# KorAP/Datok

Measured on AMD Instinct MI355X. Metric: input MB/s tokenized, tokenizer_de.matok, higher is better.
Workload: dtype u32 table cells, u8 symbol codes; 1 GPU; tokenizer_de.matok, 4096 equal-length 4096 B synthetic German docs per batch (BASELINE.json configs[1]); table_layout=matrix: state-major fused u32 cells, docs_per_gpu=4096, doc_bytes=4096, parallelism=documents sharded over 1 GPU(s), no data-path collective, batches_in_flight=3, inputs=one per batch in flight (generator seeds 2, 3, 4 on rank 0)

## Files before the change

datok_amd/csrc/dtk_batch.cpp:

```cpp
#include <algorithm>
#include <cstdio>
#include <cstring>
#include <memory>

#include "dtk_host.h"

static int alloc_outputs(dtk_batch *b, uint64_t tok, uint64_t sent, uint64_t text) {
  auto grow = [](auto &a, uint64_t n) { return a.fit(n, std::max<uint64_t>(n, 4)); };
  int rc;
  if (tok > b->tok_cap) {
    b->tok_cap = 0;
    if ((rc = grow(b->d_rstart, tok)) || (rc = grow(b->d_rend, tok)) || (rc = grow(b->d_bstart, tok)) ||
        (rc = grow(b->d_bend, tok)) || (rc = grow(b->d_sbefore, tok)))
      return rc;
    b->tok_cap = tok;
  }
  if (sent > b->sent_cap) {
    b->sent_cap = 0;
    if ((rc = grow(b->d_sent, sent))) return rc;
    b->sent_cap = sent;
  }
  if (text > b->text_cap) {
    b->text_cap = 0;
    if ((rc = grow(b->d_ttok, text)) || (rc = grow(b->d_tsent, text)) || (rc = grow(b->d_ts_end, text))) return rc;
// ... 245 lines not shown
  put(b->d_seg_tab, seg_doc.data(), (size_t)ns * 4);
  put(b->d_seg_tab + b->seg_cap, seg_lane0.data(), (size_t)ns * 4);
  put(b->d_seg_tab + 2 * (size_t)b->seg_cap, seg_nl.data(), (size_t)ns * 4);
  put(b->d_seg_tab + 3 * (size_t)b->seg_cap, doc_seg0.data(), ((size_t)nd + 1) * 4);
  put(b->d_lane_doc, lane_doc.data(), lanes * 4);
  put(b->d_chunk_off, chunk_off.data(), ((size_t)nd + 1) * 4);
  { const int rc_ = flush(); if (rc_ != DTK_OK) return rc_; }
  b->n_lanes = (uint32_t)lanes;
  b->plan_valid = true;
  return DTK_OK;
}

DtkSym sym_of(const dtk_batch *b) {
  const dtk_model *m = b->last_model;
  return DtkSym{b->d_sym, (m && m->sig.n_codes) ? m->sig.code_entry : nullptr};
}

DtkWalkArgs walk_args(dtk_batch *b) {
  DtkWalkArgs w{};
  w.sym = sym_of(b); w.doc_off = b->d_off; w.n_docs = b->n_docs;
  w.bits = b->d_bits; w.bit_words = b->bit_words; w.doc_tail = b->d_doc_tail; w.status = b->d_status;
  w.tok_cnt = b->d_tok_cnt; w.sent_cnt = b->d_sent_cnt; w.text_cnt = b->d_text_cnt;
  w.steps = (unsigned long long *)dtk_step_stripe(b->d_totals, 0);
  w.step_factor = 2048;
  return w;
}

static DtkSpecArgs spec_args(dtk_batch *b, bool redo) {
  DtkSpecArgs s{};
  s.n_lanes = b->n_lanes; s.chunk = b->chunk; s.warm = b->cfg_warm;
  s.lane_doc = b->d_lane_doc; s.chunk_off = b->d_chunk_off;
  s.lane_start = b->d_lane_start; s.lane_end = b->d_lane_end; s.lane_plan = b->d_lane_plan;
  s.lane_cnt = b->d_lane_cnt; s.first_bad = b->d_first_bad; s.fail_lane = b->d_fail_lane;
  s.redo_from = redo ? b->d_redo : nullptr;
  s.text = b->d_text;
  s.warm_extend = b->cfg_extend;
  const bool lds = g_dbg.lds_bits != 0;
  s.lds_words = (lds && b->chunk <= DTK_LDS_BIT_CHUNK_MAX) ? DTK_LDS_BIT_WORDS(b->chunk) : 0u;
  return s;
}

static uint32_t *n_bad_now(dtk_batch *b) { return b->d_totals->n_bad + b->dev_rounds; }

static int reread_flags(dtk_batch *b) {
  HIP_TRY(hipMemcpyAsync(&b->h_totals->any_irregular, &b->d_totals->any_irregular, 8, hipMemcpyDeviceToHost, b->stream));
  HIP_TRY(hipStreamSynchronize(b->stream));
  return DTK_OK;
}

static uint32_t cmp_mask_of(const dtk_model *m) {
  return LANE_F_SENT | LANE_F_TEXT | (m->unknown_used ? LANE_F_OK : 0u);
}

static int launch_compact2(dtk_batch *b, int which) {
  DtkCompactArgs a = b->last_args;
  set_outputs(b, a);
  a.tok_cap = b->tok_cap; a.sent_cap = b->sent_cap; a.text_cap = b->text_cap;
  const bool seg = b->chunk != 0 && b->long_docs;
  a.seg_doc = seg ? b->d_seg_tab : nullptr;
  a.seg_lane0 = b->d_seg_tab + b->seg_cap; a.seg_nl = b->d_seg_tab + 2 * (size_t)b->seg_cap;
  a.n_segs = b->n_segs; a.chunk_off = b->d_chunk_off; a.lane_start = b->d_lane_start; a.lane_cnt = b->d_lane_cnt;
  a.seg_sum = b->d_seg_sum; a.seg_in = b->d_seg_in;
  a.doc_seq = b->d_seg_tab + 3 * (size_t)b->seg_cap + b->max_docs + 1;
  a.any_irregular = &b->d_totals->any_irregular;
  a.any_eot = &b->d_totals->any_eot;
  b->last_args = a;
  if (seg && (which & 1) && dtk_launch_seg_prepare(&a, b->d_seg_tab + 3 * (size_t)b->seg_cap, b->stream))
    return hip_fail(hipGetLastError(), "segment carries");
  if (dtk_launch_compact(&a, b->small_max, b->d_big_docs, b->n_big, which, b->stream))
    return hip_fail(hipGetLastError(), "compact pass 2");
  if (which & 2) b->ran_full = true;
  return DTK_OK;
}

static int repair_round(dtk_batch *b, const dtk_model *m, const DtkWalkArgs *w, const DtkSpecArgs *sp, uint32_t *n_bad_out) {
  hipStream_t s = b->stream;
  if (dtk_launch_spec(&m->tab, w, sp, 5, cmp_mask_of(m), b->d_redo, n_bad_out, s) ||
      dtk_launch_redo_clear(w, sp, s))
    return hip_fail(hipGetLastError(), "speculative repair");
  for (int stage = 1; stage <= 4; stage++)
    if (dtk_launch_spec(&m->tab, w, sp, stage, cmp_mask_of(m), b->d_redo, n_bad_out, s))
      return hip_fail(hipGetLastError(), "speculative repair");
  return DTK_OK;
}


extern "C" int dtk_batch_run(const dtk_model *m, dtk_batch *b, uint32_t flags) {
  if (!m || !b) return DTK_E_ARG;
  if (b->n_docs == 0 || !b->d_off) return DTK_E_STATE;
  if (m->device != b->device) return DTK_E_ARG;
  int prc = plan_lanes(b);
  if (prc != DTK_OK) return prc;
  if (b->dl_begun && !b->dl_waited) { HIP_TRY(hipEventSynchronize(b->ev_dl)); b->dl_waited = true; }
  b->dl_begun = false;
  b->blk_pending = b->blk_failed = 0;
  b->evl_pending = false; b->evl_need = 0;
  if (b->up_pending) {
    HIP_TRY(hipStreamWaitEvent(b->stream, b->ev_up, 0));
    b->up_pending = false;
  }
  b->last_model = m;
  b->last_flags = flags;
  b->repair_rounds = 0;
  hipStream_t s = b->stream;
  const bool prof = b->profiling;
#define STAGE(i) do { if (prof) HIP_TRY(hipEventRecord(b->ev[i], s)); } while (0)
  STAGE(0);
  bool fold_acc = false;
  size_t acc_bytes = 0;
  {
    const size_t nd = b->n_docs;
    uint8_t *q = b->d_acc;
    b->d_tok_off = b->d_csr; b->d_sent_off = b->d_csr + (nd + 1); b->d_text_off = b->d_csr + 2 * (nd + 1);
    b->d_totals = (DtkTotalsDev *)q; q += DTK_TOTALS_BYTES;
    b->d_tok_cnt = (uint64_t *)q; q += (nd + 1) * 8;
    b->d_sent_cnt = (uint64_t *)q; q += (nd + 1) * 8;
    b->d_text_cnt = (uint64_t *)q; q += (nd + 1) * 8;
    b->d_status = (uint32_t *)q; q += nd * 4;
    b->d_first_bad = (uint32_t *)q; q += nd * 4;
    b->d_fail_lane = (uint32_t *)q; q += nd * 4;
    b->d_doc_tail = (uint32_t *)q; q += nd * 4;
    const size_t acc_used = ((size_t)(q - b->d_acc) + 15) & ~(size_t)15;
    b->bit_words = (uint32_t)(((b->total + nd) / 32 + 8) & ~(uint64_t)3);
    const bool fold = b->total > 0;
    fold_acc = fold && b->acc_primed && acc_used / 16 < 0xFFFFFFFFull && !g_dbg.clear_kernel;
    if (!fold_acc) {
      if (dtk_launch_clear2(b->d_acc, acc_used, b->d_bits, fold ? 0 : (size_t)EVB_KINDS * b->bit_words * 4, s))
        return hip_fail(hipGetLastError(), "clear");
      b->acc_primed = true;
    }
    acc_bytes = acc_used;
  }
  STAGE(1);
  if (dtk_launch_symbolize(b->d_text, b->d_off, b->n_docs, b->total, &m->sig, b->d_sym,
                           b->d_text == b->d_text_own, b->d_blk_doc, (unsigned long long *)&b->d_totals->invalid_epoch,
                           (uint32_t *)b->d_rsbits.p, b->d_bits, b->bit_words, fold_acc ? b->d_acc.p : nullptr, acc_bytes,
                           ++b->epoch, s))
    return hip_fail(hipGetLastError(), "symbolize");
  STAGE(2);
  DtkWalkArgs w = walk_args(b);
  bool fix_in_scan = false;
  DtkSpecArgs sp_first{};
  if (b->chunk == 0) {
    STAGE(3); STAGE(4);
    if (dtk_launch_walk(&m->tab, &w, s)) return hip_fail(hipGetLastError(), "walk");
    STAGE(5); STAGE(6); STAGE(7);
  } else {
    DtkSpecArgs sp = spec_args(b, false);
    sp_first = sp;
    uint32_t *nb = b->d_totals->n_bad;
    const bool split = g_dbg.split_start != 0 || sp.lds_words == 0;
    b->dev_rounds = g_dbg.dev_rounds >= 0 ? (uint32_t)g_dbg.dev_rounds : (b->expect_repairs ? 2u : 0u);
    if (b->dev_rounds > 3u) b->dev_rounds = 3u;
    fix_in_scan = b->n_docs <= 8192u && b->dev_rounds == 0;
#define SPEC(stage)                                                                               \
  do {                                                                                            \
    if (dtk_launch_spec(&m->tab, &w, &sp, stage, cmp_mask_of(m), b->d_redo, nb, s))               \
      return hip_fail(hipGetLastError(), "speculative walk");                                     \
  } while (0)
    if (split) {
      SPEC(0); STAGE(3); SPEC(1); STAGE(4); SPEC(2); STAGE(5); SPEC(3); STAGE(6);
    } else {
      STAGE(3); STAGE(4); SPEC(6); STAGE(5); SPEC(7); STAGE(6);
    }
    if (!fix_in_scan) SPEC(4);
    STAGE(7);
#undef SPEC
    for (uint32_t r = 0; r < b->dev_rounds; r++) {
      DtkSpecArgs rp = spec_args(b, true);
      rp.go = nb + r;
      int rc = repair_round(b, m, &w, &rp, nb + r + 1);
      if (rc != DTK_OK) return rc;
    }
  }
  DtkCompactArgs c{};
  c.text = b->d_text; c.rs_bits = (const uint32_t *)b->d_rsbits.p; c.doc_off = b->d_off; c.n_docs = b->n_docs;
  c.bits = b->d_bits; c.bit_words = b->bit_words; c.doc_tail = b->d_doc_tail; c.status = b->d_status;
  c.flags = flags & DTK_NEWLINE_AFTER_EOT; c.kind = m->kind;
  c.totals = &b->d_totals->n_tok;
  if (dtk_launch_scan3(b->d_tok_cnt, b->d_sent_cnt, b->d_text_cnt, b->d_tok_off, b->d_sent_off, b->d_text_off,
                       b->n_docs, &b->d_totals->n_tok, b->d_status, b->d_scan_ws, fix_in_scan ? &sp_first : nullptr, b->d_redo,
                       b->d_totals->n_bad, b->chunk ? n_bad_now(b) : nullptr, s))
    return hip_fail(hipGetLastError(), "scan");
  STAGE(8);
  c.skip_if = b->chunk ? n_bad_now(b) : nullptr;
  b->last_args = c;
  b->ran_full = false;
  const bool eager_full = g_dbg.compact_full != 0;
  int rc = launch_compact2(b, (b->expect_eot || eager_full) ? 3 : 1);
  if (rc != DTK_OK) return rc;
  STAGE(9);
#undef STAGE
  b->eager_fields = 0;
  b->results_changed = false;
  if (b->fields & DTK_R_EAGER) {
    rc = launch_to_host(b);
    if (rc != DTK_OK) return rc;
  }
  HIP_TRY(hipMemcpyAsync(b->h_totals, b->d_totals, DTK_TOTALS_BYTES, hipMemcpyDeviceToHost, s));
  if ((rc = b->ev_ran.ensure(hipEventDisableTiming)) != DTK_OK) return rc;
  HIP_TRY(hipEventRecord(b->ev_ran, s));
  b->ev_ran_valid = true;
  b->ran = true;
  b->totals_valid = false;
  b->render_flags = 0xFFFFFFFFu;
  return DTK_OK;
}

extern "C" int dtk_batch_done(dtk_batch *b) {
  if (!b || !b->ran || !b->ev_ran) return 0;
  const hipError_t e = hipEventQuery(b->ev_ran);
  if (e != hipSuccess) (void)hipGetLastError();
  return e == hipSuccess ? 1 : 0;
}

extern "C" int dtk_batch_set_profiling(dtk_batch *b, int enable) {
  if (!b) return DTK_E_ARG;
  if (enable)
    for (Event &e : b->ev)
      if (const int rc = e.ensure(hipEventDefault)) return rc;
  b->profiling = enable != 0;
  return DTK_OK;
}

extern "C" int dtk_batch_stage_ms(dtk_batch *b, float ms[DTK_N_STAGES]) {
  if (!b || !ms) return DTK_E_ARG;
  if (!b->ran || !b->profiling) return DTK_E_STATE;
  HIP_TRY(hipStreamSynchronize(b->stream));
  for (int i = 0; i < DTK_N_STAGES; i++) HIP_TRY(hipEventElapsedTime(&ms[i], b->ev[i], b->ev[i + 1]));
  return DTK_OK;
}

extern "C" int dtk_batch_sync(dtk_batch *b) {
  if (!b) return DTK_E_ARG;
  return wait_own(b);
}

static int run_exact(dtk_batch *b) {
  const dtk_model *m = b->last_model;
  hipStream_t s = b->stream;
  const uint32_t nd = b->n_docs;
  std::vector<uint32_t> st(nd);
  HIP_TRY(hipMemcpy(st.data(), b->d_status, (size_t)nd * 4, hipMemcpyDeviceToHost));
  for (uint32_t d = 0; d < nd; d++)
    if (st[d] & ST_IRREGULAR) b->h_exact_ids.push_back(d);
  const uint32_t n = (uint32_t)b->h_exact_ids.size();
  if (n == 0) return DTK_OK;
  if (n > b->exact_cap) {
    const uint64_t cap = (uint64_t)n + n / 4 + 16;
    int rc;
    b->exact_cap = 0;
    if ((rc = b->d_exact_ids.fit(cap, cap)) || (rc = b->d_exact_cnt.fit(cap, cap)) || (rc = b->d_exact_off.fit(cap + 1, cap + 1)))
      return rc;
    b->exact_cap = (uint32_t)cap;
  }
  HIP_TRY(hipMemcpy(b->d_exact_ids, b->h_exact_ids.data(), (size_t)n * 4, hipMemcpyHostToDevice));
  DtkExactArgs X{};
  X.sym = sym_of(b); X.text = b->d_text; X.doc_off = b->d_off; X.n = n; X.docs = b->d_exact_ids;
  X.n_calls = b->d_exact_cnt; X.call_off = b->d_exact_off; X.status = b->d_status;
  X.flags = b->last_flags & DTK_NEWLINE_AFTER_EOT; X.step_factor = walk_args(b).step_factor;
  set_outputs(b, X);
  X.pass = 0;
  if (dtk_launch_exact(&m->tab, &X, s)) return hip_fail(hipGetLastError(), "exact pass (count)");
  std::vector<uint32_t> cnt(n);
  HIP_TRY(hipMemcpyAsync(cnt.data(), b->d_exact_cnt, (size_t)n * 4, hipMemcpyDeviceToHost, s));
  HIP_TRY(hipStreamSynchronize(s));
  b->h_exact_off.assign((size_t)n + 1, 0);
  for (uint32_t i = 0; i < n; i++) b->h_exact_off[i + 1] = b->h_exact_off[i] + cnt[i];
  const uint64_t total = b->h_exact_off[n];
  if (const int rc = b->d_calls.fit(total, total + total / 4 + 16)) return rc;
  HIP_TRY(hipMemcpy(b->d_exact_off, b->h_exact_off.data(), ((size_t)n + 1) * 8, hipMemcpyHostToDevice));
  X.calls = b->d_calls;
  X.pass = 1;
  if (dtk_launch_exact(&m->tab, &X, s)) return hip_fail(hipGetLastError(), "exact pass");
  b->h_calls.resize((size_t)total);
  if (total) HIP_TRY(hipMemcpyAsync(b->h_calls.data(), b->d_calls, (size_t)total * sizeof(DtkCall), hipMemcpyDeviceToHost, s));
  HIP_TRY(hipMemcpyAsync(st.data(), b->d_status, (size_t)nd * 4, hipMemcpyDeviceToHost, s));
  HIP_TRY(hipStreamSynchronize(s));
  uint64_t flagged = 0;
  for (uint32_t d = 0; d < nd; d++) flagged += st[d] != 0;
  b->h_totals->n_flagged = flagged;
  return DTK_OK;
}

int finish(dtk_batch *b) {
  if (!b->ran) return DTK_E_STATE;
  if (b->totals_valid) return DTK_OK;
  { const int rc_ = wait_own(b); if (rc_ != DTK_OK) return rc_; }
  if (b->chunk != 0) {
    const uint32_t *hnb = b->h_totals->n_bad;
    for (uint32_t r = 0; r < b->dev_rounds; r++)
      if (hnb[r] != 0) b->repair_rounds++;
    uint32_t left = hnb[b->dev_rounds];
    if (left != 0) {
      b->results_changed = true;
      const dtk_model *m = b->last_model;
      hipStream_t s = b->stream;
      DtkWalkArgs w = walk_args(b);
      uint32_t *n_bad = n_bad_now(b);
      const uint32_t max_rounds = b->max_doc_lanes + 16u;
      while (left != 0) {
        b->repair_rounds++;
        DtkSpecArgs sp = spec_args(b, true);
        HIP_TRY(hipMemsetAsync(n_bad, 0, 4, s));
        int rc = repair_round(b, m, &w, &sp, n_bad);
        if (rc != DTK_OK) return rc;
        HIP_TRY(hipMemcpyAsync(&left, n_bad, 4, hipMemcpyDeviceToHost, s));
// ... 131 lines not shown
```

datok_amd/csrc/dtk_compact.hip:

```cpp
#include "dtk_device.h"


#define CQ_CAP 512u
#define CT_CAP 512u

struct SegRange { uint32_t d, p0, p1; bool first, last; };
__device__ __forceinline__ bool seg_range(const DtkCompactArgs &A, uint32_t s, uint32_t len_of_d, SegRange &r) {
  const uint32_t La = A.seg_lane0[s], Lb = La + A.seg_nl[s];
  const uint32_t L0 = A.chunk_off[r.d], L1 = A.chunk_off[r.d + 1];
  r.first = La == L0;
  r.last = Lb >= L1;
  r.p0 = r.first ? 0u : A.lane_start[La].p;
  if (r.p0 == 0xFFFFFFFFu) return false;
  r.p1 = r.last ? len_of_d : A.lane_start[Lb].p;
  if (r.p1 == 0xFFFFFFFFu) { r.p1 = len_of_d; r.last = true; }
  return true;
}

__device__ __forceinline__ uint32_t bits32(const uint32_t *__restrict__ b, uint32_t bit) {
  const uint32_t w = bit >> 5, sh = bit & 31u;
  const uint32_t lo = b[w], hi = b[w + 1];
  return (uint32_t)((((uint64_t)hi << 32) | lo) >> sh);
}
__device__ __forceinline__ uint32_t lowmask(uint32_t n) { return n >= 32u ? 0xFFFFFFFFu : (1u << n) - 1u; }
// ... 572 lines not shown
  for (uint32_t q0 = 0; q0 <= len; q0 += 32u) {
    const uint32_t valid = lowmask(len + 1u - q0);
    const uint32_t wE = nE & valid, wS = nS & valid, wP = nP & valid, wT = nT & valid, wU = nU & valid;
    const uint32_t wR = q0 < len ? nR & lowmask(len - q0) : 0u;
    {
      const uint32_t q1 = q0 + 32u <= len ? q0 + 32u : q0;
      nE = bits32(bE, gb + q1); nS = bits32(bS, gb + q1); nP = bits32(bP, gb + q1);
      nT = bits32(bT, gb + q1); nU = bits32(bU, gb + q1);
      nR = bits32(A.rs_bits, (uint32_t)off + (q1 < len ? q1 : 0u));
    }
    uint32_t ev = wE | wP | wT;
    while (ev) {
      const uint32_t b = (uint32_t)__ffs((int)ev) - 1u, m = 1u << b;
      ev &= ev - 1u;
      const uint32_t p = q0 + b, R = Rw + (uint32_t)__popc(wR & lowmask(b));
      if (wT & m) {
        if (wU & m) sentence_end();
        text_end();
        if (is_matrix) { B = p; RB = R; }
      }
      if (wE & m) {
        const uint32_t ms = wS & lowmask(b);
        if (ms) {
          const uint32_t sb = 31u - (uint32_t)__clz((int)ms);
          cs = q0 + sb; Rcs = Rw + (uint32_t)__popc(wR & lowmask(sb));
        }
        if (posC == 0 && nl_rule && p > B && txt[B] == '\n' && !init) posC--;
        init = false;
        posC += (int32_t)(Rcs - RB);
        const int32_t rs = posC;
        if (sentB) {
          sentB = false;
          if (n_sent < sent_n) A.sent[sent_base + n_sent] = rs; else st |= ST_INTERNAL;
          n_sent++;
        }
        posC += (int32_t)(R - Rcs);
        last_rend = posC;
        if (n_tok < tok_n) {
          if (A.tok_bstart) { A.tok_bstart[tok_base + n_tok] = cs; A.tok_bend[tok_base + n_tok] = p; }
          if (A.tok_rstart) { A.tok_rstart[tok_base + n_tok] = rs; A.tok_rend[tok_base + n_tok] = posC; }
          if (A.tok_sbefore) A.tok_sbefore[tok_base + n_tok] = n_sev;
        } else st |= ST_INTERNAL;
        n_tok++;
        B = p; RB = R;
      }
      if (wP & m) sentence_end();
    }
    if (wS) {
      const uint32_t sb = 31u - (uint32_t)__clz((int)wS);
      cs = q0 + sb; Rcs = Rw + (uint32_t)__popc(wR & lowmask(sb));
    }
    Rw += (uint32_t)__popc(wR);
  }
  if (tw & DTK_TAIL_S) sentence_end();
  if (tw & DTK_TAIL_E) text_end();
  if (st || n_tok != tok_n || n_sent != sent_n || n_text != text_n) {
    atomicOr(&A.status[d], ST_IRREGULAR);
    atomicOr(A.any_irregular, 1u);
  }
  if (A.doc_ns) A.doc_ns[d] = n_sev;
}


__device__ __forceinline__ uint32_t wave_sum(uint32_t v) {
#pragma unroll
  for (int o = 32; o > 0; o >>= 1) v += __shfl_xor(v, o);
  return v;
}

__device__ __forceinline__ uint32_t runes_between(const uint32_t *__restrict__ bits, uint64_t g0, uint64_t g1) {
  uint32_t n = 0;
  if (g1 > g0) {
    const uint64_t w0 = g0 >> 5, wl = (g1 - 1) >> 5;
    for (uint64_t w = w0 + lane_id(); w <= wl; w += WAVE) {
      uint32_t x = bits[w];
      if (w == w0) x &= 0xFFFFFFFFu << (g0 & 31u);
      if (w == wl && (g1 & 31u)) x &= (1u << (g1 & 31u)) - 1u;
      n += (uint32_t)__popc(x);
    }
  }
  return wave_sum(n);
}

__global__ __launch_bounds__(WAVE) void k_seg_sum(DtkCompactArgs A) {
  const uint32_t s = blockIdx.x;
  if (s >= A.n_segs) return;
  if (A.skip_if && *A.skip_if != 0u) return;
  const uint32_t d = A.seg_doc[s];
  if (A.chunk_off[d + 1] - A.chunk_off[d] <= DTK_SEG_LANES) return;
  const uint64_t off = A.doc_off[d];
  const uint32_t len = (uint32_t)(A.doc_off[d + 1] - off);
  const uint32_t lane = lane_id();
  DtkSegSum o{0u, 0u, 0u, 0u, 0u, 0xFFFFFFFFu, 0u, 0u};
  SegRange sr{d, 0u, len, true, true};
  if (seg_range(A, s, len, sr)) {
    const uint32_t La = A.seg_lane0[s], nl = A.seg_nl[s];
    DtkLaneCount c{0u, 0u, 0u, 0u, 0u, 0xFFFFFFFFu, 0u, 0u};
    if (lane < nl) c = A.lane_cnt[La + lane];
    uint32_t tot;
    const uint32_t tok_before = wave_excl_scan(c.tok, tot);
    o.tok = tot;
    o.sent = wave_sum(c.sent); o.text = wave_sum(c.text); o.sev = wave_sum(c.sev);
    o.runes = runes_between(A.rs_bits, off + sr.p0, off + sr.p1);
    const unsigned long long mE = __ballot(c.e_pos != 0xFFFFFFFFu);
    if (mE) {
      const int j = highest(mE);
      o.e_pos = __shfl(c.e_pos, j);
      o.e_tok = __shfl(tok_before + c.e_tok, j);
      o.e_runes = runes_between(A.rs_bits, off + sr.p0, off + o.e_pos);
    }
  }
  if (lane == 0) A.seg_sum[s] = o;
}

__global__ __launch_bounds__(WAVE) void k_seg_scan(DtkCompactArgs A, const uint32_t *doc_seg0) {
  const uint32_t d = blockIdx.x;
  if (d >= A.n_docs) return;
  if (A.skip_if && *A.skip_if != 0u) return;
  const uint32_t s0 = doc_seg0[d], s1 = doc_seg0[d + 1];
  if (s1 - s0 <= 1u) return;
  const uint32_t lane = lane_id();
  bool any_e = false;
  uint32_t bt = 0, bs = 0, bx = 0, bv = 0, br = 0;
  uint32_t ce_pos = 0xFFFFFFFFu, ce_tok = 0, ce_runes = 0;
  for (uint32_t g = s0; g < s1; g += WAVE) {
    const uint32_t s = g + lane;
    DtkSegSum v{0u, 0u, 0u, 0u, 0u, 0xFFFFFFFFu, 0u, 0u};
    if (s < s1) v = A.seg_sum[s];
    uint32_t tt, ts, tx, tv, tr;
    const uint32_t et = wave_excl_scan(v.tok, tt), es = wave_excl_scan(v.sent, ts), ex = wave_excl_scan(v.text, tx);
    const uint32_t ev = wave_excl_scan(v.sev, tv), er = wave_excl_scan(v.runes, tr);
    const unsigned long long mE = __ballot(v.e_pos != 0xFFFFFFFFu);
    const unsigned long long below = mE & lanemask_lt();
    const int j = below ? highest(below) : 0;
    const uint32_t jp = __shfl(v.e_pos, j), jt = __shfl(bt + et + v.e_tok, j), jr = __shfl(br + er + v.e_runes, j);
    if (s < s1) {
      DtkSegIn in;
      in.tok = bt + et; in.sent = bs + es; in.text = bx + ex; in.sev = bv + ev; in.runes = br + er;
      in.e_pos = below ? jp : ce_pos; in.e_tok = below ? jt : ce_tok; in.e_runes = below ? jr : ce_runes;
      A.seg_in[s] = in;
    }
    if (mE) {
      const int jl = highest(mE);
      ce_pos = __shfl(v.e_pos, jl); ce_tok = __shfl(bt + et + v.e_tok, jl); ce_runes = __shfl(br + er + v.e_runes, jl);
      any_e = true;
    }
    bt += tt; bs += ts; bx += tx; bv += tv; br += tr;
  }
  if (lane == 0) A.doc_seq[d] = (A.kind != DTK_KIND_MATRIX && any_e) ? 1u : 0u;
}



#define SCAN1_TB 1024u
__global__ __launch_bounds__(SCAN1_TB) void k_scan3(const uint64_t *ca, const uint64_t *cb, const uint64_t *cc,
                                                uint64_t *a, uint64_t *b, uint64_t *c, uint32_t n,
                                                uint64_t *totals, const uint32_t *status, DtkSpecArgs S,
                                                uint32_t *redo_out, uint32_t *n_bad, int fix, const uint32_t *skip_if) {
  if (skip_if && *skip_if != 0u) return;
  __shared__ uint64_t wsum[3][SCAN1_TB / WAVE];
  __shared__ uint32_t wfl[SCAN1_TB / WAVE];
  const uint32_t T = blockDim.x, tid = threadIdx.x, lane = tid & 63u, wid = tid >> 6;
  const uint32_t per = (n + T - 1) / T;
  const uint32_t lo = tid * per < n ? tid * per : n;
  const uint32_t hi = lo + per < n ? lo + per : n;
  uint64_t sa = 0, sb = 0, sc = 0;
  uint32_t fl = 0;
  constexpr uint32_t G = 4u;
  for (uint32_t i0 = lo; i0 < hi; i0 += G) {
    uint64_t va[G], vb[G], vc[G];
    uint32_t vs[G], vf[G];
#pragma unroll
    for (uint32_t j = 0; j < G; j++) {
      const uint32_t i = i0 + j;
      const bool ok = i < hi;
      va[j] = ok ? ca[i] : 0ull; vb[j] = ok ? cb[i] : 0ull; vc[j] = ok ? cc[i] : 0ull;
      vs[j] = ok ? status[i] : 0u;
      vf[j] = (ok && fix) ? S.fail_lane[i] : 0u;
    }
#pragma unroll
    for (uint32_t j = 0; j < G; j++) {
      sa += va[j]; sb += vb[j]; sc += vc[j]; fl += vs[j] != 0u;
      if (fix && i0 + j < hi) {
        const uint32_t bad = ~vf[j];
        if (bad == 0xFFFFFFFFu) redo_out[i0 + j] = 0xFFFFFFFFu; else mark_redo(S, i0 + j, bad, redo_out, n_bad);
      }
    }
  }
  uint64_t xa = sa, xb = sb, xc = sc;
  uint32_t xf = fl;
#pragma unroll
  for (int o = 1; o < WAVE; o <<= 1) {
    const uint64_t ya = __shfl_up(xa, o), yb = __shfl_up(xb, o), yc = __shfl_up(xc, o);
    const uint32_t yf = __shfl_up(xf, o);
    if ((int)lane >= o) { xa += ya; xb += yb; xc += yc; xf += yf; }
  }
  if (lane == WAVE - 1) { wsum[0][wid] = xa; wsum[1][wid] = xb; wsum[2][wid] = xc; wfl[wid] = xf; }
  __syncthreads();
  uint64_t ba = 0, bb = 0, bc = 0;
  uint32_t bf = 0;
  for (uint32_t w = 0; w < wid; w++) { ba += wsum[0][w]; bb += wsum[1][w]; bc += wsum[2][w]; bf += wfl[w]; }
  uint64_t ra = ba + xa - sa, rb = bb + xb - sb, rc = bc + xc - sc;
  for (uint32_t i0 = lo; i0 < hi; i0 += G) {
    uint64_t va[G], vb[G], vc[G];
#pragma unroll
    for (uint32_t j = 0; j < G; j++) {
      const uint32_t i = i0 + j;
      const bool ok = i < hi;
      va[j] = ok ? ca[i] : 0ull; vb[j] = ok ? cb[i] : 0ull; vc[j] = ok ? cc[i] : 0ull;
    }
#pragma unroll
    for (uint32_t j = 0; j < G; j++) {
      const uint32_t i = i0 + j;
      if (i < hi) { a[i] = ra; b[i] = rb; c[i] = rc; }
      ra += va[j]; rb += vb[j]; rc += vc[j];
    }
  }
  if (tid == T - 1) {
    a[n] = ba + xa; b[n] = bb + xb; c[n] = bc + xc;
    totals[0] = ba + xa; totals[1] = bb + xb; totals[2] = bc + xc;
    totals[3] = bf + xf;
  }
}

#ifndef DTK_TOHOST_WAVES
#define DTK_TOHOST_WAVES 128u
#endif
__global__ __launch_bounds__(WAVE) void k_to_host(DtkToHostArgs A) {
  if (A.skip_if && *A.skip_if != 0u) return;
  bool fits = true;
  for (uint32_t i = 0; i < A.n; i++)
    if (A.count_from[i] >= 0 && A.totals[A.count_from[i]] > A.cap[i]) fits = false;
  if (!fits) return;
  const uint32_t lane = threadIdx.x;
  for (uint32_t i = 0; i < A.n; i++) {
    const uint64_t bytes = A.count_from[i] >= 0 ? A.totals[A.count_from[i]] * A.bytes[i] : A.bytes[i];
    const uint4 *__restrict__ s16 = reinterpret_cast<const uint4 *>(A.src[i]);
    uint4 *__restrict__ d16 = reinterpret_cast<uint4 *>(A.dst[i]);
    const uint64_t n16 = bytes >> 4;
    for (uint64_t p = (blockIdx.x + gridDim.x - i % gridDim.x) % gridDim.x; p * WAVE < n16; p += gridDim.x) {
      const uint64_t j = p * WAVE + lane;
      if (j < n16) {
        const uint4 v = s16[j];
        d16[j] = v;
      }
      asm volatile("s_waitcnt vmcnt(0)" ::: "memory");
    }
    if (blockIdx.x == i % gridDim.x && lane < (bytes & 15u))
      reinterpret_cast<uint8_t *>(A.dst[i])[(n16 << 4) + lane] = reinterpret_cast<const uint8_t *>(A.src[i])[(n16 << 4) + lane];
  }
  if (blockIdx.x == 0 && lane == 0) *A.done = A.epoch;
}

extern "C" int dtk_launch_to_host(const DtkToHostArgs *args, void *stream) {
  hipLaunchKernelGGL(k_to_host, dim3(DTK_TOHOST_WAVES), dim3(WAVE), 0, (hipStream_t)stream, *args);
  return (int)hipGetLastError();
}

__global__ __launch_bounds__(256) void k_pack_r16(const int32_t *__restrict__ rs, const int32_t *__restrict__ re,
                                                  uint32_t *__restrict__ out, uint64_t n) {
  const uint64_t i4 = ((uint64_t)blockIdx.x * 256u + threadIdx.x) * 4u;
  if (i4 + 4u <= n) {
    const int4 a = *reinterpret_cast<const int4 *>(rs + i4), b = *reinterpret_cast<const int4 *>(re + i4);
    *reinterpret_cast<uint4 *>(out + i4) =
        make_uint4(((uint32_t)a.x & 0xFFFFu) | ((uint32_t)b.x << 16), ((uint32_t)a.y & 0xFFFFu) | ((uint32_t)b.y << 16),
                   ((uint32_t)a.z & 0xFFFFu) | ((uint32_t)b.z << 16), ((uint32_t)a.w & 0xFFFFu) | ((uint32_t)b.w << 16));
  } else {
    for (uint64_t i = i4; i < n; i++) out[i] = ((uint32_t)rs[i] & 0xFFFFu) | ((uint32_t)re[i] << 16);
  }
}

extern "C" int dtk_launch_pack_r16(const int32_t *rs, const int32_t *re, uint32_t *out, uint64_t n, void *stream) {
  if (n == 0) return 0;
  hipLaunchKernelGGL(k_pack_r16, dim3((unsigned)((n + 1023u) / 1024u)), dim3(256), 0, (hipStream_t)stream, rs, re, out, n);
  return (int)hipGetLastError();
}

__global__ __launch_bounds__(256) void k_pack_blk(DtkPackBlkArgs A) {
  const DtkPackBlkPair P = A.pair[blockIdx.y];
  const uint32_t lane = lane_id();
  const uint64_t blk = (uint64_t)blockIdx.x * 4u + (threadIdx.x >> 6);
  if (blk * WAVE >= A.n) return;
  const uint64_t i = blk * WAVE + lane;
  const bool live = i < A.n;
  int32_t s = 0, e = 0;
  if (live) { s = P.start[i]; e = P.end[i]; }
  const int32_t prev_e = __shfl_up(e, 1);
  const unsigned long long dec = __ballot(live && lane != 0u && s < prev_e);
  const uint32_t brk = dec ? (uint32_t)__ffsll((long long)dec) - 1u : (uint32_t)WAVE;
  const bool seg1 = lane >= brk;
  const int32_t lo = live ? min(s, e) : INT32_MAX, hi = live ? max(s, e) : INT32_MIN;
  const int32_t lo0 = wave_min(seg1 ? INT32_MAX : lo), hi0 = wave_max(seg1 ? INT32_MIN : hi);
  int32_t lo1 = 0, hi1 = 0;
  if (brk < WAVE) { lo1 = wave_min(seg1 ? lo : INT32_MAX); hi1 = wave_max(seg1 ? hi : INT32_MIN); }
  const int32_t base = seg1 ? lo1 : lo0;
  if (live) P.words[i] = ((uint32_t)(s - base) & 0xFFFFu) | ((uint32_t)(e - base) << 16);
  if (lane == 0u) {
    reinterpret_cast<uint4 *>(P.heads)[blk] = make_uint4((uint32_t)lo0, (uint32_t)lo1, brk, 0u);
    if ((int64_t)hi0 - lo0 > (int64_t)A.span || (int64_t)hi1 - lo1 > (int64_t)A.span) atomicOr(P.flag, 1u);
  }
}

extern "C" int dtk_launch_pack_blk(const DtkPackBlkArgs *args, void *stream) {
  if (args->n == 0 || args->n_pairs == 0) return 0;
  const uint64_t blocks = (args->n + WAVE - 1) / WAVE;
  hipLaunchKernelGGL(k_pack_blk, dim3((unsigned)((blocks + 3u) / 4u), args->n_pairs), dim3(256), 0, (hipStream_t)stream, *args);
  return (int)hipGetLastError();
}


__global__ __launch_bounds__(256) void k_clear2(uint4 *__restrict__ a, uint64_t na16, uint4 *__restrict__ b,
                                                uint64_t nb16) {
  const uint64_t stride = (uint64_t)gridDim.x * blockDim.x;
  const uint4 z = make_uint4(0u, 0u, 0u, 0u);
  for (uint64_t i = (uint64_t)blockIdx.x * blockDim.x + threadIdx.x; i < na16 + nb16; i += stride) {
    if (i < na16) a[i] = z; else b[i - na16] = z;
  }
}

extern "C" int dtk_launch_clear2(void *a, uint64_t a_bytes, void *b, uint64_t b_bytes, void *stream) {
  const uint64_t n16 = (a_bytes + b_bytes) / 16;
  if (n16 == 0) return 0;
  uint64_t blocks = (n16 + 256ull * 4 - 1) / (256ull * 4);
  if (blocks > 8192) blocks = 8192;
  hipLaunchKernelGGL(k_clear2, dim3((uint32_t)blocks), dim3(256), 0, (hipStream_t)stream, (uint4 *)a, a_bytes / 16,
                     (uint4 *)b, b_bytes / 16);
  return (int)hipGetLastError();
}

extern "C" int dtk_launch_compact(const DtkCompactArgs *args, uint32_t small_max, const uint32_t *big_docs, uint32_t n_big,
                                  int which, void *stream) {
  if (args->n_docs == 0) return 0;
  hipStream_t s = (hipStream_t)stream;
  if (small_max && (which & 1))
    hipLaunchKernelGGL(k_compact_small, dim3((args->n_docs + 255u) / 256u), dim3(256), 0, s, *args, small_max);
  const uint32_t grid = args->seg_doc ? args->n_segs : (small_max ? n_big : args->n_docs);
  const uint32_t *list = args->seg_doc ? nullptr : (small_max ? big_docs : nullptr);
  if (grid && (which & 1)) hipLaunchKernelGGL(k_compact_plain, dim3(grid), dim3(WAVE), 0, s, *args, small_max, list);
  if (grid && (which & 2)) hipLaunchKernelGGL(k_compact_eot, dim3(grid), dim3(WAVE), 0, s, *args, small_max, list);
  return (int)hipGetLastError();
}

extern "C" int dtk_launch_seg_prepare(const DtkCompactArgs *args, const uint32_t *doc_seg0, void *stream) {
  hipStream_t s = (hipStream_t)stream;
  hipLaunchKernelGGL(k_seg_sum, dim3(args->n_segs), dim3(WAVE), 0, s, *args);
  hipLaunchKernelGGL(k_seg_scan, dim3(args->n_docs), dim3(WAVE), 0, s, *args, doc_seg0);
  return (int)hipGetLastError();
}

#define SCAN_TB 256u
#define SCAN_PER 8u
#define SCAN_TILE (SCAN_TB * SCAN_PER)

__device__ __forceinline__ uint64_t scan_block_excl(uint64_t v, uint64_t *sh, uint64_t &total) {
  const uint32_t tid = threadIdx.x;
  sh[tid] = v;
  __syncthreads();
  for (uint32_t o = 1; o < SCAN_TB; o <<= 1) {
    const uint64_t x = tid >= o ? sh[tid - o] : 0;
    __syncthreads();
    sh[tid] += x;
    __syncthreads();
  }
  total = sh[SCAN_TB - 1];
  const uint64_t ex = sh[tid] - v;
  __syncthreads();
  return ex;
}

__global__ __launch_bounds__(SCAN_TB) void k_scan3_sums(const uint64_t *ca, const uint64_t *cb, const uint64_t *cc,
                                                        const uint32_t *status, uint32_t n, uint64_t *ws, const uint32_t *skip_if) {
  if (skip_if && *skip_if != 0u) return;
  __shared__ uint64_t sh[SCAN_TB];
  const uint32_t i0 = blockIdx.x * SCAN_TILE + threadIdx.x * SCAN_PER;
  uint64_t s[4] = {0, 0, 0, 0};
  for (uint32_t i = i0; i < i0 + SCAN_PER && i < n; i++) { s[0] += ca[i]; s[1] += cb[i]; s[2] += cc[i]; s[3] += status[i] != 0; }
  for (int j = 0; j < 4; j++) {
    uint64_t tot;
    (void)scan_block_excl(s[j], sh, tot);
    if (threadIdx.x == 0) ws[4u * blockIdx.x + j] = tot;
  }
}

__global__ __launch_bounds__(SCAN_TB) void k_scan3_mid(uint64_t *ws, uint32_t nb, uint64_t *a, uint64_t *b, uint64_t *c,
                                                       uint32_t n, uint64_t *totals, const uint32_t *skip_if) {
  if (skip_if && *skip_if != 0u) return;
  __shared__ uint64_t sh[SCAN_TB];
  const uint32_t tid = threadIdx.x;
  const uint32_t per = (nb + SCAN_TB - 1) / SCAN_TB;
  const uint32_t lo = min(tid * per, nb), hi = min(lo + per, nb);
  for (int j = 0; j < 4; j++) {
    uint64_t sm = 0;
    for (uint32_t i = lo; i < hi; i++) sm += ws[4u * i + j];
    uint64_t tot;
    uint64_t run = scan_block_excl(sm, sh, tot);
    for (uint32_t i = lo; i < hi; i++) { const uint64_t v = ws[4u * i + j]; ws[4u * i + j] = run; run += v; }
    if (tid == 0) {
      totals[j] = tot;
      if (j == 0) a[n] = tot;
      if (j == 1) b[n] = tot;
      if (j == 2) c[n] = tot;
    }
  }
}

__global__ __launch_bounds__(SCAN_TB) void k_scan3_apply(const uint64_t *ca, const uint64_t *cb, const uint64_t *cc,
                                                         uint64_t *a, uint64_t *b, uint64_t *c, uint32_t n,
                                                         const uint64_t *ws, const uint32_t *skip_if) {
  if (skip_if && *skip_if != 0u) return;
  __shared__ uint64_t sh[SCAN_TB];
  const uint32_t i0 = blockIdx.x * SCAN_TILE + threadIdx.x * SCAN_PER;
  const uint64_t *src[3] = {ca, cb, cc};
  uint64_t *dst[3] = {a, b, c};
  for (int j = 0; j < 3; j++) {
    uint64_t v[SCAN_PER], sm = 0;
    for (uint32_t q = 0; q < SCAN_PER; q++) { v[q] = i0 + q < n ? src[j][i0 + q] : 0; sm += v[q]; }
    uint64_t tot;
    uint64_t run = ws[4u * blockIdx.x + j] + scan_block_excl(sm, sh, tot);
    for (uint32_t q = 0; q < SCAN_PER; q++) {
      if (i0 + q < n) dst[j][i0 + q] = run;
      run += v[q];
    }
  }
}

extern "C" int dtk_launch_scan3(const uint64_t *ca, const uint64_t *cb, const uint64_t *cc, uint64_t *a,
                                uint64_t *b, uint64_t *c, uint32_t n_docs, uint64_t *totals,
                                const uint32_t *status, uint64_t *ws, const DtkSpecArgs *fix_spec,
                                uint32_t *redo_out, uint32_t *n_bad, const uint32_t *skip_if, void *stream) {
  hipStream_t s = (hipStream_t)stream;
  if (n_docs <= 8192u || !ws) {
    DtkSpecArgs none{};
    hipLaunchKernelGGL(k_scan3, dim3(1), dim3(SCAN1_TB), 0, s, ca, cb, cc, a, b, c, n_docs, totals, status,
                       fix_spec ? *fix_spec : none, redo_out, n_bad, fix_spec ? 1 : 0, skip_if);
  } else {
    if (fix_spec) return -1;
    const uint32_t nb = (n_docs + SCAN_TILE - 1) / SCAN_TILE;
    hipLaunchKernelGGL(k_scan3_sums, dim3(nb), dim3(SCAN_TB), 0, s, ca, cb, cc, status, n_docs, ws, skip_if);
    hipLaunchKernelGGL(k_scan3_mid, dim3(1), dim3(SCAN_TB), 0, s, ws, nb, a, b, c, n_docs, totals, skip_if);
    hipLaunchKernelGGL(k_scan3_apply, dim3(nb), dim3(SCAN_TB), 0, s, ca, cb, cc, a, b, c, n_docs, ws, skip_if);
  }
  return (int)hipGetLastError();
}
```

datok_amd/csrc/dtk_device.h:

```cpp
#pragma once
#include <hip/hip_runtime.h>
#include <stdint.h>

#include <type_traits>

#include "dtk_internal.h"

#define WAVE 64
#ifndef DTK_WARM_TAG
#define DTK_WARM_TAG 64u
#endif


__device__ __forceinline__ uint32_t lane_id() { return threadIdx.x & (WAVE - 1); }
__device__ __forceinline__ unsigned long long lanemask_lt() { return (1ull << lane_id()) - 1ull; }
__device__ __forceinline__ int highest(unsigned long long m) { return 63 - __clzll((long long)m); }
__device__ __forceinline__ uint32_t popc(unsigned long long m) { return (uint32_t)__popcll(m); }

__device__ __forceinline__ uint32_t wave_excl_scan(uint32_t v, uint32_t &total) {
  uint32_t x = v;
  x += (uint32_t)__builtin_amdgcn_update_dpp(0, (int)x, 0x111, 0xF, 0xF, true);
  x += (uint32_t)__builtin_amdgcn_update_dpp(0, (int)x, 0x112, 0xF, 0xF, true);
  x += (uint32_t)__builtin_amdgcn_update_dpp(0, (int)x, 0x114, 0xF, 0xF, true);
  x += (uint32_t)__builtin_amdgcn_update_dpp(0, (int)x, 0x118, 0xF, 0xF, true);
  x += (uint32_t)__builtin_amdgcn_update_dpp(0, (int)x, 0x142, 0xA, 0xF, false);
  x += (uint32_t)__builtin_amdgcn_update_dpp(0, (int)x, 0x143, 0xC, 0xF, false);
  total = (uint32_t)__builtin_amdgcn_readlane((int)x, WAVE - 1);
  return x - v;
}

#define DTK_WAVE_FOLD(x, op)                                                                   \
  do {                                                                                         \
    x = op(x, __builtin_amdgcn_update_dpp(x, x, 0x111, 0xF, 0xF, false));       \
    x = op(x, __builtin_amdgcn_update_dpp(x, x, 0x112, 0xF, 0xF, false));       \
    x = op(x, __builtin_amdgcn_update_dpp(x, x, 0x114, 0xF, 0xF, false));       \
    x = op(x, __builtin_amdgcn_update_dpp(x, x, 0x118, 0xF, 0xF, false));       \
    x = op(x, __builtin_amdgcn_update_dpp(x, x, 0x142, 0xA, 0xF, false));    \
    x = op(x, __builtin_amdgcn_update_dpp(x, x, 0x143, 0xC, 0xF, false));    \
  } while (0)
__device__ __forceinline__ int32_t wave_min(int32_t v) {
  int x = v;
  DTK_WAVE_FOLD(x, min);
  return __builtin_amdgcn_readlane(x, WAVE - 1);
}
__device__ __forceinline__ int32_t wave_max(int32_t v) {
  int x = v;
  DTK_WAVE_FOLD(x, max);
  return __builtin_amdgcn_readlane(x, WAVE - 1);
}

__device__ __forceinline__ uint32_t doc_of(const uint64_t *__restrict__ doc_off, uint32_t lo, uint32_t hi,
                                           uint64_t g) {
  while (hi - lo > 1) {
    const uint32_t mid = lo + ((hi - lo) >> 1);
    if (doc_off[mid] <= g) lo = mid; else hi = mid;
  }
  return lo;
}

__device__ __forceinline__ void mark_redo(const DtkSpecArgs &S, uint32_t d, uint32_t bad, uint32_t *redo_out,
                                          uint32_t *n_bad) {
  const uint32_t L0 = S.chunk_off[d], L1 = S.chunk_off[d + 1];
  DtkLaneState en = S.lane_end[bad];
  en.flags &= (LANE_F_SENT | LANE_F_TEXT | LANE_F_OK);
  if (en.p != 0xFFFFFFFFu && bad + 1 < L1) S.lane_start[bad + 1] = en;
  uint32_t r0 = bad;
  if (bad > L0) {
    r0 = bad - 1u;
    while (r0 > L0 && S.lane_end[r0].p == S.lane_start[r0].p) r0--;
  }
  redo_out[d] = r0;
  atomicAdd(n_bad, 1u);
}
```

datok_amd/csrc/dtk_internal.h:

```cpp
#pragma once
#include <stddef.h>
#include <stdint.h>

#define DTK_FIRSTBIT 0x80000000u
#define DTK_SECONDBIT 0x40000000u
#define DTK_RESTBIT 0x3fffffffu
#define DTK_EOT 4u
#define DTK_WINDOW 1024u
#define DTK_WINDOW_BYTES 4104u

#define DTK_SYM_MASK 0x7FFu
#define DTK_SYM_MAX 2047u
#define DTK_SYM_W_SHIFT 11
#define DTK_SYM_CLS_SHIFT 14
#define DTK_SYM_WIDTH(e) (((uint32_t)(e) >> DTK_SYM_W_SHIFT) & 7u)
#define DTK_SYM_IS_START(e) (DTK_SYM_WIDTH(e) != 0u)
#define DTK_WIN 32u
#define DTK_WIN_ROW 36u
#define DTK_SYM_CONT 0xFFu
#ifndef DTK_WIN8
#define DTK_WIN8 32u
#endif
#ifndef DTK_WIN16
#define DTK_WIN16 16u
// ... 166 lines not shown
  uint32_t flags;
  int kind;
  uint64_t *tok_off, *sent_off, *text_off;
  int32_t *tok_rstart, *tok_rend;
  uint32_t *tok_bstart, *tok_bend;
  int32_t *sent;
  uint32_t *text_tok_end, *text_sent_end;
  uint32_t *tok_sbefore, *text_s_end, *doc_ns;
  const uint64_t *totals;
  uint64_t tok_cap, sent_cap, text_cap;
  const uint32_t *seg_doc, *seg_lane0, *seg_nl;
  uint32_t n_segs;
  const uint32_t *chunk_off;
  const struct DtkLaneState *lane_start;
  const struct DtkLaneCount *lane_cnt;
  struct DtkSegSum *seg_sum;
  struct DtkSegIn *seg_in;
  uint32_t *doc_seq;
  uint32_t *any_irregular;
  uint32_t *any_eot;
  const uint32_t *skip_if;
};

#define DTK_SEG_LANES 64u
struct DtkSegSum {
  uint32_t tok, sent, text, sev;
  uint32_t runes;
  uint32_t e_pos;
  uint32_t e_tok, e_runes;
};
struct DtkSegIn {
  uint32_t tok, sent, text, sev, runes;
  uint32_t e_pos, e_tok, e_runes;
};

struct DtkCall { uint32_t kind; int32_t a; uint32_t b, c; };
struct DtkExactArgs {
  struct DtkSym sym;
  const uint8_t *text;
  const uint64_t *doc_off;
  uint32_t n;
  const uint32_t *docs;
  uint32_t pass;
  uint32_t *n_calls;
  const uint64_t *call_off;
  struct DtkCall *calls;
  uint32_t *status;
  uint32_t flags;
  uint32_t step_factor;
  const uint64_t *tok_off, *sent_off, *text_off;
  int32_t *tok_rstart, *tok_rend;
  uint32_t *tok_bstart, *tok_bend;
  int32_t *sent;
  uint32_t *text_tok_end, *text_sent_end;
  uint32_t *tok_sbefore, *text_s_end, *doc_ns;
};

struct DtkRenderArgs {
  const uint8_t *text;
  const uint64_t *doc_off;
  uint32_t n_docs;
  uint32_t flags;
  const uint64_t *tok_off, *sent_off, *text_off;
  uint64_t n_tok, n_sent, n_text;
  const int32_t *rstart, *rend, *sent;
  const uint32_t *bstart, *bend, *sbefore;
  const uint32_t *ttok, *tsent, *ts_end;
  const uint32_t *doc_ns;
  struct DtkSym sym;
  uint64_t *A, *P, *Q;
  uint64_t *blkA, *blkP, *blkQ;
  uint64_t *ns_off;
  uint64_t *tx_base, *tx_stream, *tx_pos, *tx_sent;
  uint64_t *out_off;
  uint8_t *out;
  uint64_t out_total;
};

#define DTK_TOHOST_MAX 14
struct DtkToHostArgs {
  const void *src[DTK_TOHOST_MAX];
  void *dst[DTK_TOHOST_MAX];
  uint64_t bytes[DTK_TOHOST_MAX];
  int32_t count_from[DTK_TOHOST_MAX];
  uint64_t cap[DTK_TOHOST_MAX];
  uint32_t n;
  const uint64_t *totals;
  const uint32_t *skip_if;
  uint64_t *done;
  uint64_t epoch;
};

struct DtkPackBlkPair {
  const int32_t *start, *end;
  uint32_t *words;
  void *heads;
  uint32_t *flag;
};
struct DtkPackBlkArgs {
  struct DtkPackBlkPair pair[2];
  uint32_t n_pairs;
  uint32_t span;
  uint64_t n;
};

#define DTK_EVL_K_SEOT 1u
#define DTK_EVL_K_TEOT 2u
#define DTK_EVL_K_SEPS 4u
struct DtkEvListArgs {
  const uint32_t *bits;
  uint32_t bit_words;
  uint32_t n_docs;
  const uint64_t *doc_off;
  uint64_t n_bits;
  uint32_t n_tiles;
  uint32_t cap;
  uint32_t *tile_base;
  uint32_t *count;
  uint32_t *evl_off;
  uint32_t *evl_pos;
  uint8_t *evl_kind;
  uint32_t *evl_bit;
};

#ifdef __cplusplus
extern "C" {
#endif
uint32_t dtk_evlist_tiles(uint64_t n_bits, uint32_t bit_words);
int dtk_launch_evlist(const struct DtkEvListArgs *args, void *stream);
int dtk_launch_to_host(const struct DtkToHostArgs *args, void *stream);
int dtk_launch_pack_r16(const int32_t *rs, const int32_t *re, uint32_t *out, uint64_t n, void *stream);
int dtk_launch_pack_blk(const struct DtkPackBlkArgs *args, void *stream);
int dtk_launch_symbolize(const uint8_t *text, const uint64_t *doc_off, uint32_t n_docs,
                         uint64_t total, const struct DtkSigmaDev *sig, void *sym, int padded,
                         const uint32_t *blk_doc, unsigned long long *n_invalid, uint32_t *rs_bits,
                         uint32_t *ev_bits, uint32_t bit_words, void *acc, uint64_t acc_bytes, uint64_t epoch, void *stream);
#ifndef DTK_SYM_BLOCK_BYTES
#define DTK_SYM_BLOCK_BYTES 4096u
#endif
int dtk_launch_walk(const struct DtkTableDev *tab, const struct DtkWalkArgs *args, void *stream);
int dtk_launch_spec(const struct DtkTableDev *tab, const struct DtkWalkArgs *args,
                    const struct DtkSpecArgs *spec, int stage, uint32_t cmp_mask, uint32_t *redo_out,
                    uint32_t *n_bad, void *stream);
int dtk_launch_spec_check(const struct DtkWalkArgs *args, const struct DtkSpecArgs *spec, int stage, uint32_t cmp_mask,
                          uint32_t *redo_out, uint32_t *n_bad, void *stream);
int dtk_launch_redo_clear(const struct DtkWalkArgs *args, const struct DtkSpecArgs *spec, void *stream);
int dtk_launch_compact(const struct DtkCompactArgs *args, uint32_t small_max, const uint32_t *big_docs, uint32_t n_big,
                       int which, void *stream);
int dtk_launch_exact(const struct DtkTableDev *tab, const struct DtkExactArgs *args, void *stream);
int dtk_launch_seg_prepare(const struct DtkCompactArgs *args, const uint32_t *doc_seg0, void *stream);
int dtk_launch_render(const struct DtkRenderArgs *args, int stage, void *stream);
uint32_t dtk_render_tiles(uint64_t n);
int dtk_launch_clear2(void *a, uint64_t a_bytes, void *b, uint64_t b_bytes, void *stream);
int dtk_launch_scan3(const uint64_t *ca, const uint64_t *cb, const uint64_t *cc, uint64_t *a, uint64_t *b,
                     uint64_t *c, uint32_t n_docs, uint64_t *totals, const uint32_t *status, uint64_t *ws,
                     const struct DtkSpecArgs *fix_spec, uint32_t *redo_out, uint32_t *n_bad, const uint32_t *skip_if,
                     void *stream);
#ifdef __cplusplus
}
#endif
```

Baseline: 180,400 MB/s.

## Replace single-block doc scan with multi-block tile scan using redundant prefix sums

The small-batch scan of per-document token, sentence and text counts, which also applies fail-lane fixes, used to run in one 1024-thread block. It now runs as a grid of 256-thread tiles. Each tile recomputes the sum of all earlier documents itself with strided loads, so no inter-block synchronisation is needed, then uses wave shuffle scans for the in-tile prefix. The shared block scan helper is also changed from a log-step shared-memory scan to a wave-shuffle scan. The cost is redundant reading of earlier elements, which grows quadratically with the number of docs. The skip_if early exit is now bypassed whenever fix is set.

Measured after the change: 191,000 MB/s (median of 6 runs). 5.9% higher.

```diff
diff --git a/datok_amd/csrc/dtk_batch.cpp b/datok_amd/csrc/dtk_batch.cpp
--- a/datok_amd/csrc/dtk_batch.cpp
+++ b/datok_amd/csrc/dtk_batch.cpp
@@ -421,7 +421,7 @@
     const bool split = g_dbg.split_start != 0 || sp.lds_words == 0;
     b->dev_rounds = g_dbg.dev_rounds >= 0 ? (uint32_t)g_dbg.dev_rounds : (b->expect_repairs ? 2u : 0u);
     if (b->dev_rounds > 3u) b->dev_rounds = 3u;
-    fix_in_scan = b->n_docs <= 8192u && b->dev_rounds == 0;
+    fix_in_scan = b->n_docs <= DTK_SCAN_TILES_MAX_DOCS && b->dev_rounds == 0;
 #define SPEC(stage)                                                                               \
   do {                                                                                            \
     if (dtk_launch_spec(&m->tab, &w, &sp, stage, cmp_mask_of(m), b->d_redo, nb, s))               \
diff --git a/datok_amd/csrc/dtk_compact.hip b/datok_amd/csrc/dtk_compact.hip
--- a/datok_amd/csrc/dtk_compact.hip
+++ b/datok_amd/csrc/dtk_compact.hip
@@ -748,74 +748,80 @@
 
 
 
-#define SCAN1_TB 1024u
-__global__ __launch_bounds__(SCAN1_TB) void k_scan3(const uint64_t *ca, const uint64_t *cb, const uint64_t *cc,
-                                                uint64_t *a, uint64_t *b, uint64_t *c, uint32_t n,
-                                                uint64_t *totals, const uint32_t *status, DtkSpecArgs S,
-                                                uint32_t *redo_out, uint32_t *n_bad, int fix, const uint32_t *skip_if) {
-  if (skip_if && *skip_if != 0u) return;
-  __shared__ uint64_t wsum[3][SCAN1_TB / WAVE];
-  __shared__ uint32_t wfl[SCAN1_TB / WAVE];
-  const uint32_t T = blockDim.x, tid = threadIdx.x, lane = tid & 63u, wid = tid >> 6;
-  const uint32_t per = (n + T - 1) / T;
-  const uint32_t lo = tid * per < n ? tid * per : n;
-  const uint32_t hi = lo + per < n ? lo + per : n;
-  uint64_t sa = 0, sb = 0, sc = 0;
-  uint32_t fl = 0;
-  constexpr uint32_t G = 4u;
-  for (uint32_t i0 = lo; i0 < hi; i0 += G) {
+#define SCAN_TB 256u
+
+__device__ __forceinline__ uint64_t scan_block_excl(uint64_t v, uint64_t *sh, uint64_t &total) {
+  const uint32_t lane = lane_id(), wid = threadIdx.x >> 6;
+  const uint64_t x = wave_incl_scan64(v);
+  if (lane == WAVE - 1) sh[wid] = x;
+  __syncthreads();
+  uint64_t base = 0, tot = 0;
+#pragma unroll
+  for (uint32_t w = 0; w < SCAN_TB / WAVE; w++) {
+    const uint64_t s = sh[w];
+    if (w < wid) base += s;
+    tot += s;
+  }
+  __syncthreads();
+  total = tot;
+  return base + x - v;
+}
+
+__global__ __launch_bounds__(SCAN_TB) void k_scan3_tiles(const uint64_t *ca, const uint64_t *cb, const uint64_t *cc,
+                                                         uint64_t *a, uint64_t *b, uint64_t *c, uint32_t n,
+                                                         uint64_t *totals, const uint32_t *status, DtkSpecArgs S,
+                                                         uint32_t *redo_out, uint32_t *n_bad, int fix,
+                                                         const uint32_t *skip_if) {
+  if (!fix && skip_if && *skip_if != 0u) return;
+  constexpr uint32_t NW = SCAN_TB / WAVE;
+  __shared__ uint64_t wsum[2][3][NW];
+  __shared__ uint32_t wfl[2][NW];
+  const uint32_t tid = threadIdx.x, lane = tid & 63u, wid = tid >> 6;
+  const uint32_t below = blockIdx.x * SCAN_TB, i = below + tid;
+  const bool last = blockIdx.x == gridDim.x - 1, in = i < n;
+  const uint64_t ma = in ? ca[i] : 0ull, mb = in ? cb[i] : 0ull, mc = in ? cc[i] : 0ull;
+  const uint32_t ms = in ? status[i] : 0u;
+  const uint32_t mf = (in && fix) ? S.fail_lane[i] : 0u;
+  uint64_t pa = 0, pb = 0, pc = 0;
+  uint32_t pf = 0;
+  constexpr uint32_t G = 8u;
+  for (uint32_t j0 = tid; j0 < below; j0 += G * SCAN_TB) {
     uint64_t va[G], vb[G], vc[G];
-    uint32_t vs[G], vf[G];
+    uint32_t vs[G];
 #pragma unroll
-    for (uint32_t j = 0; j < G; j++) {
-      const uint32_t i = i0 + j;
-      const bool ok = i < hi;
-      va[j] = ok ? ca[i] : 0ull; vb[j] = ok ? cb[i] : 0ull; vc[j] = ok ? cc[i] : 0ull;
-      vs[j] = ok ? status[i] : 0u;
-      vf[j] = (ok && fix) ? S.fail_lane[i] : 0u;
+    for (uint32_t q = 0; q < G; q++) {
+      const uint32_t j = j0 + q * SCAN_TB;
+      const bool ok = j < below;
+      va[q] = ok ? ca[j] : 0ull; vb[q] = ok ? cb[j] : 0ull; vc[q] = ok ? cc[j] : 0ull;
+      vs[q] = (ok && last) ? status[j] : 0u;
     }
 #pragma unroll
-    for (uint32_t j = 0; j < G; j++) {
-      sa += va[j]; sb += vb[j]; sc += vc[j]; fl += vs[j] != 0u;
-      if (fix && i0 + j < hi) {
-        const uint32_t bad = ~vf[j];
-        if (bad == 0xFFFFFFFFu) redo_out[i0 + j] = 0xFFFFFFFFu; else mark_redo(S, i0 + j, bad, redo_out, n_bad);
-      }
-    }
-  }
-  uint64_t xa = sa, xb = sb, xc = sc;
-  uint32_t xf = fl;
-#pragma unroll
-  for (int o = 1; o < WAVE; o <<= 1) {
-    const uint64_t ya = __shfl_up(xa, o), yb = __shfl_up(xb, o), yc = __shfl_up(xc, o);
-    const uint32_t yf = __shfl_up(xf, o);
-    if ((int)lane >= o) { xa += ya; xb += yb; xc += yc; xf += yf; }
-  }
-  if (lane == WAVE - 1) { wsum[0][wid] = xa; wsum[1][wid] = xb; wsum[2][wid] = xc; wfl[wid] = xf; }
+    for (uint32_t q = 0; q < G; q++) { pa += va[q]; pb += vb[q]; pc += vc[q]; pf += vs[q] != 0u; }
+  }
+  const uint64_t xa = wave_incl_scan64(ma), xb = wave_incl_scan64(mb), xc = wave_incl_scan64(mc);
+  const uint64_t ya = wave_incl_scan64(pa), yb = wave_incl_scan64(pb), yc = wave_incl_scan64(pc);
+  const uint32_t xf = popc(__ballot(ms != 0u)), yf = wave_sum(pf);
+  if (lane == WAVE - 1) {
+    wsum[0][0][wid] = ya; wsum[0][1][wid] = yb; wsum[0][2][wid] = yc; wfl[0][wid] = yf;
+    wsum[1][0][wid] = xa; wsum[1][1][wid] = xb; wsum[1][2][wid] = xc; wfl[1][wid] = xf;
+  }
   __syncthreads();
   uint64_t ba = 0, bb = 0, bc = 0;
   uint32_t bf = 0;
-  for (uint32_t w = 0; w < wid; w++) { ba += wsum[0][w]; bb += wsum[1][w]; bc += wsum[2][w]; bf += wfl[w]; }
-  uint64_t ra = ba + xa - sa, rb = bb + xb - sb, rc = bc + xc - sc;
-  for (uint32_t i0 = lo; i0 < hi; i0 += G) {
-    uint64_t va[G], vb[G], vc[G];
 #pragma unroll
-    for (uint32_t j = 0; j < G; j++) {
-      const uint32_t i = i0 + j;
-      const bool ok = i < hi;
-      va[j] = ok ? ca[i] : 0ull; vb[j] = ok ? cb[i] : 0ull; vc[j] = ok ? cc[i] : 0ull;
-    }
-#pragma unroll
-    for (uint32_t j = 0; j < G; j++) {
-      const uint32_t i = i0 + j;
-      if (i < hi) { a[i] = ra; b[i] = rb; c[i] = rc; }
-      ra += va[j]; rb += vb[j]; rc += vc[j];
-    }
-  }
-  if (tid == T - 1) {
+  for (uint32_t w = 0; w < NW; w++) {
+    ba += wsum[0][0][w]; bb += wsum[0][1][w]; bc += wsum[0][2][w]; bf += wfl[0][w] + wfl[1][w];
+    if (w < wid) { ba += wsum[1][0][w]; bb += wsum[1][1][w]; bc += wsum[1][2][w]; }
+  }
+  if (in) { a[i] = ba + xa - ma; b[i] = bb + xb - mb; c[i] = bc + xc - mc; }
+  if (last && tid == SCAN_TB - 1u) {
     a[n] = ba + xa; b[n] = bb + xb; c[n] = bc + xc;
     totals[0] = ba + xa; totals[1] = bb + xb; totals[2] = bc + xc;
-    totals[3] = bf + xf;
+    totals[3] = bf;
+  }
+  if (fix && in) {
+    const uint32_t bad = ~mf;
+    if (bad == 0xFFFFFFFFu) redo_out[i] = 0xFFFFFFFFu; else mark_redo(S, i, bad, redo_out, n_bad);
   }
 }
 
@@ -944,30 +950,13 @@
   return (int)hipGetLastError();
 }
 
-#define SCAN_TB 256u
 #define SCAN_PER 8u
 #define SCAN_TILE (SCAN_TB * SCAN_PER)
-
-__device__ __forceinline__ uint64_t scan_block_excl(uint64_t v, uint64_t *sh, uint64_t &total) {
-  const uint32_t tid = threadIdx.x;
-  sh[tid] = v;
-  __syncthreads();
-  for (uint32_t o = 1; o < SCAN_TB; o <<= 1) {
-    const uint64_t x = tid >= o ? sh[tid - o] : 0;
-    __syncthreads();
-    sh[tid] += x;
-    __syncthreads();
-  }
-  total = sh[SCAN_TB - 1];
-  const uint64_t ex = sh[tid] - v;
-  __syncthreads();
-  return ex;
-}
 
 __global__ __launch_bounds__(SCAN_TB) void k_scan3_sums(const uint64_t *ca, const uint64_t *cb, const uint64_t *cc,
                                                         const uint32_t *status, uint32_t n, uint64_t *ws, const uint32_t *skip_if) {
   if (skip_if && *skip_if != 0u) return;
-  __shared__ uint64_t sh[SCAN_TB];
+  __shared__ uint64_t sh[SCAN_TB / WAVE];
   const uint32_t i0 = blockIdx.x * SCAN_TILE + threadIdx.x * SCAN_PER;
   uint64_t s[4] = {0, 0, 0, 0};
   for (uint32_t i = i0; i < i0 + SCAN_PER && i < n; i++) { s[0] += ca[i]; s[1] += cb[i]; s[2] += cc[i]; s[3] += status[i] != 0; }
@@ -981,7 +970,7 @@
 __global__ __launch_bounds__(SCAN_TB) void k_scan3_mid(uint64_t *ws, uint32_t nb, uint64_t *a, uint64_t *b, uint64_t *c,
                                                        uint32_t n, uint64_t *totals, const uint32_t *skip_if) {
   if (skip_if && *skip_if != 0u) return;
-  __shared__ uint64_t sh[SCAN_TB];
+  __shared__ uint64_t sh[SCAN_TB / WAVE];
   const uint32_t tid = threadIdx.x;
   const uint32_t per = (nb + SCAN_TB - 1) / SCAN_TB;
   const uint32_t lo = min(tid * per, nb), hi = min(lo + per, nb);
@@ -1004,7 +993,7 @@
                                                          uint64_t *a, uint64_t *b, uint64_t *c, uint32_t n,
                                                          const uint64_t *ws, const uint32_t *skip_if) {
   if (skip_if && *skip_if != 0u) return;
-  __shared__ uint64_t sh[SCAN_TB];
+  __shared__ uint64_t sh[SCAN_TB / WAVE];
   const uint32_t i0 = blockIdx.x * SCAN_TILE + threadIdx.x * SCAN_PER;
   const uint64_t *src[3] = {ca, cb, cc};
   uint64_t *dst[3] = {a, b, c};
@@ -1025,9 +1014,10 @@
                                 const uint32_t *status, uint64_t *ws, const DtkSpecArgs *fix_spec,
                                 uint32_t *redo_out, uint32_t *n_bad, const uint32_t *skip_if, void *stream) {
   hipStream_t s = (hipStream_t)stream;
-  if (n_docs <= 8192u || !ws) {
+  if (n_docs <= DTK_SCAN_TILES_MAX_DOCS || !ws) {
     DtkSpecArgs none{};
-    hipLaunchKernelGGL(k_scan3, dim3(1), dim3(SCAN1_TB), 0, s, ca, cb, cc, a, b, c, n_docs, totals, status,
+    const uint32_t tiles = n_docs ? (n_docs + SCAN_TB - 1u) / SCAN_TB : 1u;
+    hipLaunchKernelGGL(k_scan3_tiles, dim3(tiles), dim3(SCAN_TB), 0, s, ca, cb, cc, a, b, c, n_docs, totals, status,
                        fix_spec ? *fix_spec : none, redo_out, n_bad, fix_spec ? 1 : 0, skip_if);
   } else {
     if (fix_spec) return -1;
diff --git a/datok_amd/csrc/dtk_device.h b/datok_amd/csrc/dtk_device.h
--- a/datok_amd/csrc/dtk_device.h
+++ b/datok_amd/csrc/dtk_device.h
@@ -27,6 +27,17 @@
   x += (uint32_t)__builtin_amdgcn_update_dpp(0, (int)x, 0x143, 0xC, 0xF, false);
   total = (uint32_t)__builtin_amdgcn_readlane((int)x, WAVE - 1);
   return x - v;
+}
+
+__device__ __forceinline__ uint64_t wave_incl_scan64(uint64_t v) {
+  const uint32_t lane = lane_id();
+  uint64_t x = v;
+#pragma unroll
+  for (uint32_t o = 1; o < WAVE; o <<= 1) {
+    const uint64_t y = __shfl_up(x, o);
+    if (lane >= o) x += y;
+  }
+  return x;
 }
 
 #define DTK_WAVE_FOLD(x, op)                                                                   \
diff --git a/datok_amd/csrc/dtk_internal.h b/datok_amd/csrc/dtk_internal.h
--- a/datok_amd/csrc/dtk_internal.h
+++ b/datok_amd/csrc/dtk_internal.h
@@ -342,6 +342,9 @@
 int dtk_launch_render(const struct DtkRenderArgs *args, int stage, void *stream);
 uint32_t dtk_render_tiles(uint64_t n);
 int dtk_launch_clear2(void *a, uint64_t a_bytes, void *b, uint64_t b_bytes, void *stream);
+#ifndef DTK_SCAN_TILES_MAX_DOCS
+#define DTK_SCAN_TILES_MAX_DOCS 8192u
+#endif
 int dtk_launch_scan3(const uint64_t *ca, const uint64_t *cb, const uint64_t *cc, uint64_t *a, uint64_t *b,
                      uint64_t *c, uint32_t n_docs, uint64_t *totals, const uint32_t *status, uint64_t *ws,
                      const struct DtkSpecArgs *fix_spec, uint32_t *redo_out, uint32_t *n_bad, const uint32_t *skip_if,
```
